# lh3/miniasm

Measured on NVIDIA H100. Metric: paf_overlaps_per_sec_ingest_to_gfa, higher is better.
Workload: dtype int64/uint32 (+3 float32 predicates)

## Files before the change

### miniasm_b200/csrc/capi_fused.cu

```cuda
#include "../../include/miniasm_b200.h"
#include "capi_util.cuh"
#include "hit_dev.cuh"
#include "clean_dev.cuh"
#include "gfa_dev.cuh"
#include "dump_dev.cuh"
#include "ugseq_dev.cuh"
#include <pthread.h>
#include "ingest_dev.cuh"
#include "shard_comm.cuh"
#include <cub/cub.cuh>
#include <map>
#include <string>
#include <zlib.h>
#include <fcntl.h>
#include <unistd.h>
#include <sys/stat.h>

ma_ug_t *mab_ug_download(MabDev &d, DUnitigs &du);
extern "C" sdict_t *sd_from_packed(char *block, size_t block_size, uint32_t n, const uint32_t *len);

struct mab_ctx {
	MabDev dev;
	char *d_text = nullptr;
	size_t text_len = 0, text_cap = 0;
// ... 279 lines not shown
	uint32_t *nl = (uint32_t*)malloc((dict->n_seq ? dict->n_seq : 1) * 4), *sl = (uint32_t*)malloc((dict->n_seq ? dict->n_seq : 1) * 4);
	bytes = 0;
	for (uint32_t i = 0; i < dict->n_seq; ++i) {
		size_t l = strlen(dict->seq[i].name);
		memcpy(pack + bytes, dict->seq[i].name, l + 1);
		off[i] = bytes, nl[i] = (uint32_t)l, sl[i] = dict->seq[i].len;
		bytes += l + 1;
	}
	text_reserve(c, bytes);
	c->text_len = bytes;
	DNames &nm = c->names;
	nm.n_seq = dict->n_seq;
	nm.off = mab_alloc<uint64_t>(d, nm.n_seq); nm.nlen = mab_alloc<uint32_t>(d, nm.n_seq); nm.slen = mab_alloc<uint32_t>(d, nm.n_seq);
	if (bytes) MAB_CUDA(cudaMemcpyAsync(c->d_text, pack, bytes, cudaMemcpyHostToDevice, d.stream));
	if (nm.n_seq) {
		MAB_CUDA(cudaMemcpyAsync(nm.off, off, (size_t)nm.n_seq * 8, cudaMemcpyHostToDevice, d.stream));
		MAB_CUDA(cudaMemcpyAsync(nm.nlen, nl, (size_t)nm.n_seq * 4, cudaMemcpyHostToDevice, d.stream));
		MAB_CUDA(cudaMemcpyAsync(nm.slen, sl, (size_t)nm.n_seq * 4, cudaMemcpyHostToDevice, d.stream));
	}
	d.sync();
	free(pack); free(off); free(nl); free(sl);
	c->n_seq = dict->n_seq;
	c->stats.n_hits_stored = n, c->stats.n_seq_in = dict->n_seq;
	return 0;
}

int mab_select(mab_ctx_t *c, const ma_opt_t *opt, int no_first, int no_second, int stage)
{
	MAB_CUDA(cudaSetDevice(c->dev.device));
	MabDev &d = c->dev;
	DHits &h = c->hits;
	PhaseTimer pt(d, &c->stats.ms_select, "mab_select");
	ctx_drop_graphs(c);
	auto step3_banner = [] { if (!mab_mute && ma_verbose >= 1) fprintf(stderr, "[M::main] ===> Step 3: 2-pass (fine) read selection <===\n"); };
	if (!no_first && !no_second && stage >= 5) {
		if (!mab_mute && ma_verbose >= 1) fprintf(stderr, "[M::main] ===> Step 2: 1-pass (crude) read selection <===\n");
		select_default(c, opt, { step3_banner });
		c->stats.n_hits_final = h.n, c->stats.n_seq_final = c->n_seq;
		d.sync();
		return 0;
	}
	if (!no_first) {
		if (!mab_mute && ma_verbose >= 1) fprintf(stderr, "[M::main] ===> Step 2: 1-pass (crude) read selection <===\n");
		if (stage >= 2) {
			d.free(c->sub);
			c->sub = mab_alloc<DSub>(d, c->n_seq);
			d.trace("select:begin");
			dh_sub(d, h, opt->min_dp, opt->min_iden, 0, c->sub);
			d.trace("select:sub1");
			dh_cut(d, h, c->sub, opt->min_span);
			if (stage >= 3) dh_flt(d, h, c->sub, (int)(opt->max_hang * 1.5), (int)(opt->min_ovlp * .5), &c->cov);
			d.trace("select:cut1(+flt)");
		}
	}
	if (!no_second) {
		step3_banner();
		if (stage >= 4) {
			DSub *sub2 = mab_alloc<DSub>(d, c->n_seq);
			d.trace("select:flt");
			dh_sub(d, h, opt->min_dp, opt->min_iden, opt->min_span / 2, sub2);
			d.trace("select:sub2");
			dh_cut(d, h, sub2, opt->min_span);
			if (!no_first && c->sub) { dh_sub_merge(d, c->n_seq, c->sub, sub2); d.free(sub2); }
			else { d.free(c->sub); c->sub = sub2; }
		}
		if (stage >= 5 && c->sub) {
// ... 110 lines not shown
	++d.n_lib;
	uint64_t last_pos; uint32_t last_sz;
	MAB_CUDA(cudaMemcpyAsync(&last_pos, pos + n - 1, 8, cudaMemcpyDeviceToHost, d.stream));
	MAB_CUDA(cudaMemcpyAsync(&last_sz, sz + n - 1, 4, cudaMemcpyDeviceToHost, d.stream));
	d.sync();
	const size_t bytes = last_pos + last_sz;
	char *d_pack = (char*)d.alloc(bytes), *pack = (char*)malloc(bytes);
	uint32_t *slen = (uint32_t*)malloc((size_t)n * 4);
	MAB_LAUNCH(d, k_name_pack, mab_grid(n, 256), 256, 0, n, c->orig_id, c->names.off, c->names.nlen, c->names.slen, c->name_text ? c->name_text : c->d_text, pos, d_pack, d_slen);
	MAB_CUDA(cudaMemcpyAsync(pack, d_pack, bytes, cudaMemcpyDeviceToHost, d.stream));
	MAB_CUDA(cudaMemcpyAsync(slen, d_slen, (size_t)n * 4, cudaMemcpyDeviceToHost, d.stream));
	d.sync();
	sd_destroy(dict);
	dict = sd_from_packed(pack, bytes, n, slen);
	free(slen);
	d.free(sz); d.free(d_slen); d.free(pos); d.free(d_pack);
	d.sync();
	return dict;
}

ma_sub_t *mab_export_sub(mab_ctx_t *c)
{
	MAB_CUDA(cudaSetDevice(c->dev.device));
	if (!c->sub) return 0;
	ma_sub_t *s = (ma_sub_t*)calloc(c->n_seq ? c->n_seq : 1, sizeof(ma_sub_t));
	if (c->n_seq) MAB_CUDA(cudaMemcpyAsync(s, c->sub, (size_t)c->n_seq * sizeof(DSub), cudaMemcpyDeviceToHost, c->dev.stream));
	c->dev.sync();
	return s;
}

ma_hit_t *mab_export_hits(mab_ctx_t *c, size_t *n)
{
	MAB_CUDA(cudaSetDevice(c->dev.device));
	ma_hit_t *a = (ma_hit_t*)malloc((c->hits.n ? c->hits.n : 1) * sizeof(ma_hit_t));
	if (c->hits.n) MAB_CUDA(cudaMemcpyAsync(a, c->hits.a, c->hits.n * sizeof(DHit), cudaMemcpyDeviceToHost, c->dev.stream));
	c->dev.sync();
	*n = c->hits.n;
	return a;
}

asg_t *mab_export_sg(mab_ctx_t *c)
{
	MAB_CUDA(cudaSetDevice(c->dev.device));
	if (!c->have_sg) return 0;
	asg_t *g = asg_init();
	g->n_seq = c->sg.n_seq, g->m_seq = c->sg.n_seq ? c->sg.n_seq : 1;
	g->seq = (asg_seq_t*)malloc((size_t)g->m_seq * sizeof(asg_seq_t));
	g->m_arc = c->sg.n_arc ? c->sg.n_arc : 1;
	g->arc = (asg_arc_t*)malloc((size_t)g->m_arc * sizeof(asg_arc_t));
	mab_graph_download(c->dev, c->sg, g);
	return g;
}

ma_ug_t *mab_export_ug(mab_ctx_t *c)
{
	MAB_CUDA(cudaSetDevice(c->dev.device));
	if (!c->have_ug) return 0;
	return mab_ug_download(c->dev, c->ug);
}

float mab_coverage(const mab_ctx_t *c) { return c->cov; }

long mab_write_gfa(mab_ctx_t *c, FILE *fp)
{
	MAB_CUDA(cudaSetDevice(c->dev.device));
	if (!c->have_ug) return -1;
	MabDev &d = c->dev;
	if (!c->ug.g.has_idx) dg_arc_index(d, c->ug.g);
	char *d_txt = nullptr;
	const size_t n = dg_gfa_text(d, c->ug, c->orig_id, c->names.off, c->names.nlen, c->name_text ? c->name_text : c->d_text, c->sub, &d_txt);
	if (n) {
		if (n > c->h_gfa_cap) {
			if (c->h_gfa) MAB_CUDA(cudaFreeHost(c->h_gfa));
			c->h_gfa_cap = n + (n >> 2) + (1 << 20);
			MAB_CUDA(cudaHostAlloc((void**)&c->h_gfa, c->h_gfa_cap, cudaHostAllocDefault));
		}
		MAB_CUDA(cudaMemcpyAsync(c->h_gfa, d_txt, n, cudaMemcpyDeviceToHost, d.stream));
		d.sync();
		if (fwrite(c->h_gfa, 1, n, fp) != n) { fprintf(stderr, "[E::miniasm_b200] short write of the GFA text\n"); exit(74); }
	}
	d.free(d_txt);
	d.sync();
	return (long)n;
}

static long write_dump(mab_ctx *c, DumpKind kind, uint64_t n_rec, FILE *fp)
{
	const DumpView v{{c->orig_id, c->names.off, c->names.nlen, c->name_text ? c->name_text : c->d_text, c->sub}, c->hits.a, c->sg.arc};
	return (long)dg_dump_write(c->dev, kind, v, n_rec, fp, c->pin, c->pin_bytes);
}

long mab_write_paf(mab_ctx_t *c, FILE *fp)
{
	MAB_CUDA(cudaSetDevice(c->dev.device));
	if (!c->sub) return -1;
	return write_dump(c, DUMP_PAF, c->hits.n, fp);
}

long mab_write_bed(mab_ctx_t *c, FILE *fp)
{
	MAB_CUDA(cudaSetDevice(c->dev.device));
	if (!c->sub) return -1;
	return write_dump(c, DUMP_BED, c->n_seq, fp);
}

long mab_write_sg(mab_ctx_t *c, FILE *fp)
{
	MAB_CUDA(cudaSetDevice(c->dev.device));
	if (!c->have_sg) return -1;
	return write_dump(c, DUMP_SG, c->sg.n_arc, fp);
}

static void *reads_loader(void *p)
{
	mab_ctx::ReadsLoad *rl = (mab_ctx::ReadsLoad*)p;
	const size_t CH = 32u << 20;
	cudaStream_t st;
	char *pin[2];
	cudaEvent_t ev[2];
	MAB_CUDA(cudaSetDevice(rl->device));
	gzFile fp = rl->fn != "-" ? gzopen(rl->fn.c_str(), "r") : gzdopen(fileno(stdin), "r");
	if (fp == 0) { rl->rc = -1; return 0; }
	gzbuffer(fp, 1 << 20);
	MAB_CUDA(cudaStreamCreateWithFlags(&st, cudaStreamNonBlocking));
	for (int i = 0; i < 2; ++i) { MAB_CUDA(cudaMallocHost(&pin[i], CH)); MAB_CUDA(cudaEventCreateWithFlags(&ev[i], cudaEventDisableTiming)); }
	struct stat sb;
	size_t guess = 0;
	if (rl->fn != "-" && stat(rl->fn.c_str(), &sb) == 0) guess = (size_t)sb.st_size;
// ... 134 lines not shown
	ctx_reset_reads(c);
	text_reserve(c, len);
	c->text_len = len;
	PhaseTimer pt(d, &c->stats.ms_ingest, "mab_load_ingest_text_sharded");
	ingest_paf_sharded(d, c->sc, c->d_text, c->text_len, min_span, min_match, bi_dir, c->hits, c->names, &c->name_text, c->ist, text);
	c->n_seq = c->names.n_seq;
	c->stats.n_lines = c->ist.n_parsed, c->stats.n_hits_stored = c->ist.n_hits, c->stats.n_seq_in = c->ist.n_seq;
	if (!mab_mute && ma_verbose >= 3 && c->sc.rank == 0)
		fprintf(stderr, "[M::%s::%s] read %ld hits; stored %ld hits and %d sequences (%ld bp)\n", "ma_hit_read", sys_timestamp(),
				(long)c->ist.n_parsed, (long)c->ist.n_hits, (int)c->ist.n_seq, (long)c->ist.tot_len);
	return 0;
}

static void sum_over_ranks(void *ctx, unsigned long long *v, int n)
{
	mab_ctx *c = (mab_ctx*)ctx;
	if (!c->sc.active() || n <= 0 || n > 8) return;
	MabDev &d = c->dev;
	unsigned long long *buf = (unsigned long long*)mab_alloc<uint64_t>(d, 8);
	MAB_CUDA(cudaMemcpyAsync(buf, v, 8 * (size_t)n, cudaMemcpyHostToDevice, d.stream));
	MAB_NCCL(ncclAllReduce(buf, buf, (size_t)n, ncclUint64, ncclSum, c->sc.comm, d.stream));
	MAB_CUDA(cudaMemcpyAsync(v, buf, 8 * (size_t)n, cudaMemcpyDeviceToHost, d.stream));
	d.sync();
	d.free(buf);
}

int mab_select_sharded(mab_ctx_t *c, const ma_opt_t *opt)
{
	MAB_CUDA(cudaSetDevice(c->dev.device));
	MabDev &d = c->dev;
	ShardComm &sc = c->sc;
	PhaseTimer pt(d, &c->stats.ms_select, "mab_select_sharded");
	ctx_drop_graphs(c);
	const int msave = mab_mute;
	if (sc.rank != 0) mab_mute = 1;
	mab_count_hook = sum_over_ranks, mab_count_hook_ctx = c;
	const uint32_t n = c->n_seq;
	SelectHooks hk;
	hk.sub_done = [&](DSub *s) { sc_allreduce(d, sc, s, n, ncclUint64, ncclSum); };
	hk.flags_done = [&](DSub *sub, uint8_t *used, uint32_t n_seq) {
		sc_allreduce(d, sc, sub, (size_t)n_seq * 2, ncclUint32, ncclMax);
		sc_allreduce(d, sc, used, n_seq, ncclUint8, ncclMax);
	};
	select_default(c, opt, hk);
	mab_mute = msave;
	mab_count_hook = nullptr, mab_count_hook_ctx = nullptr;
	c->stats.n_hits_final = c->hits.n, c->stats.n_seq_final = c->n_seq;
	d.sync();
	return 0;
}

__global__ void k_not_flag(const uint8_t *flag, uint32_t n, uint8_t *out)
{
	for (uint32_t i = blockIdx.x * blockDim.x + threadIdx.x; i < n; i += gridDim.x * blockDim.x) out[i] = !flag[i];
}

int mab_layout_sharded(mab_ctx_t *c, const ma_opt_t *opt)
{
	MAB_CUDA(cudaSetDevice(c->dev.device));
	MabDev &d = c->dev;
	ShardComm &sc = c->sc;
	const int G = sc.world;
	PhaseTimer pt(d, &c->stats.ms_layout, "mab_layout_sharded");
	ctx_drop_graphs(c);
	const int msave = mab_mute;
	if (sc.rank != 0) mab_mute = 1;
// ... 109 lines not shown
```

### miniasm_b200/csrc/hit_dev.cu

```cuda
#include "hit_dev.cuh"
#include "hit2arc.cuh"
#include <cub/cub.cuh>
#include <functional>

extern "C" int ma_verbose;
extern "C" const char *sys_timestamp(void);
#define ma_verbose_dev (mab_mute ? 0 : ma_verbose)

thread_local MabCountHook mab_count_hook = nullptr;
thread_local void *mab_count_hook_ctx = nullptr;
static inline void sum_ranks(unsigned long long *v, int n) { if (mab_count_hook) mab_count_hook(mab_count_hook_ctx, v, n); }

__device__ __forceinline__ DHit ld_hit(const DHit *p)
{
	const uint4 *q = reinterpret_cast<const uint4*>(p);
	uint4 a = __ldg(q), b = __ldg(q + 1);
	DHit h;
	h.qns = (uint64_t)a.y << 32 | a.x; h.qe = a.z; h.tn = a.w;
	h.ts = b.x; h.te = b.y; h.ml_rev = b.z; h.bl_del = b.w;
	return h;
}
__device__ __forceinline__ DHit ld_hit_rw(const DHit *p)
{
	const uint4 *q = reinterpret_cast<const uint4*>(p);
	uint4 a = q[0], b = q[1];
	DHit h;
	h.qns = (uint64_t)a.y << 32 | a.x; h.qe = a.z; h.tn = a.w;
	h.ts = b.x; h.te = b.y; h.ml_rev = b.z; h.bl_del = b.w;
	return h;
}
__device__ __forceinline__ void st_hit(DHit *p, const DHit &h)
{
	uint4 *q = reinterpret_cast<uint4*>(p);
	q[0] = make_uint4((uint32_t)h.qns, (uint32_t)(h.qns >> 32), h.qe, h.tn);
	q[1] = make_uint4(h.ts, h.te, h.ml_rev, h.bl_del);
}

static inline uint32_t bits_for(uint64_t x) { uint32_t b = 0; while (x) ++b, x >>= 1; return b ? b : 1; }

static void drop_bounds(MabDev &d, DHits &h) { d.free(h.grp); h.grp = nullptr; }

void dh_reserve(MabDev &d, DHits &h, size_t m)
{
	drop_bounds(d, h);
	if (m <= h.m) return;
	DHit *na = mab_alloc<DHit>(d, m), *nb = mab_alloc<DHit>(d, m);
	if (h.n) MAB_CUDA(cudaMemcpyAsync(na, h.a, h.n * sizeof(DHit), cudaMemcpyDeviceToDevice, d.stream));
	d.free(h.a); d.free(h.a2);
	h.a = na, h.a2 = nb, h.m = m;
}

void dh_free(MabDev &d, DHits &h)
{
	d.free(h.a); d.free(h.a2); d.free(h.grp);
	h = DHits();
}

constexpr int SEL_ROWS = 8, SEL_THREADS = 256, SEL_TILE = SEL_ROWS * SEL_THREADS;
static_assert(SEL_ROWS * (SEL_THREADS / 32) == 64, "k_sel_scatter scans exactly two counts per lane of one warp");

__global__ void __launch_bounds__(SEL_THREADS)
k_sel_count(const uint8_t *__restrict__ flag, size_t n, uint32_t *__restrict__ tile_cnt, unsigned long long *__restrict__ total)
{
	__shared__ unsigned s_w[SEL_THREADS / 32];
	const size_t base = (size_t)blockIdx.x * SEL_TILE;
	unsigned c = 0;
	#pragma unroll
	for (int k = 0; k < SEL_ROWS; ++k) {
		const size_t i = base + (size_t)k * SEL_THREADS + threadIdx.x;
		c += (i < n && flag[i] != 0) ? 1u : 0u;
	}
	c = __reduce_add_sync(0xffffffffu, c);
	if ((threadIdx.x & 31) == 0) s_w[threadIdx.x >> 5] = c;
	__syncthreads();
	if (threadIdx.x == 0) {
		unsigned t = 0;
		#pragma unroll
		for (int w = 0; w < SEL_THREADS / 32; ++w) t += s_w[w];
		tile_cnt[blockIdx.x] = t;
		if (t) atomicAdd(total, (unsigned long long)t);
	}
}

__global__ void __launch_bounds__(SEL_THREADS)
k_sel_scatter(const DHit *__restrict__ in, const uint8_t *__restrict__ flag, size_t n, const uint32_t *__restrict__ tile_off,
              DHit *__restrict__ out, unsigned long long *__restrict__ n_out)
{
// ... 1024 lines not shown
			DHit p;
			bool keep = false, dirty = false;
			if (i < end) {
				p = ld_hit_rw(a + i);
				const DHit o = p;
				const DSub rt = sub2[p.tn];
				keep = mab_cut_hit(p, rq, rt, min_span);
				if (keep) {
					dirty = hit_clipped(p, o);
					DArc tmp;
					const int rr = mab_hit2arc(p, (int)(rq.e - rq.s_del), (int)(rt.e - rt.s_del), hp.max_hang, hp.int_frac, hp.min_ovlp, &tmp);
					if (rr == MAB_HT_QCONT) atomicOr(&sub[r].s_del, MAB_DEL_BIT);
					else if (rr == MAB_HT_TCONT) atomicOr(&sub[p.tn].s_del, MAB_DEL_BIT);
					used[p.tn] = 1;
				}
			}
			const unsigned km = __ballot_sync(0xffffffffu, keep);
			const uint32_t dst = first + kept + __popc(km & lt);
			if (keep) {
				if (dst != i || dirty) st_hit(a + dst, p);
				tn_out[dst] = p.tn;
			}
			kept += __popc(km);
		}
		if (lane == 0) {
			grp[r] = kept ? (uint64_t)first << 32 | (first + kept) : 0;
			if (kept) used[r] = 1, cut += kept;
		}
	}
	if (lane == 0 && cut) atomicAdd(n_cut, (unsigned long long)cut);
}

__global__ void __launch_bounds__(256)
k_sel_final_count(const uint64_t *__restrict__ grp, const uint32_t *__restrict__ tn, const int32_t *__restrict__ map, uint32_t n_seq, uint32_t *cnt)
{
	const int lane = threadIdx.x & 31;
	for (uint32_t r = (blockIdx.x * blockDim.x + threadIdx.x) >> 5; r < n_seq; r += (gridDim.x * blockDim.x) >> 5) {
		const int32_t m = map[r];
		if (m < 0) continue;
		const uint64_t g = grp[r];
		const uint32_t end = (uint32_t)g, first = (uint32_t)(g >> 32);
		unsigned c = 0;
		if (end) for (uint32_t i = first + lane; i < end; i += 32) c += map[tn[i]] >= 0;
		c = __reduce_add_sync(0xffffffffu, c);
		if (lane == 0) cnt[m] = c;
	}
}

__global__ void __launch_bounds__(256)
k_sel_final_copy(const DHit *__restrict__ a, const uint64_t *__restrict__ grp, const int32_t *__restrict__ map, uint32_t n_seq,
                 const uint32_t *__restrict__ off, const uint32_t *__restrict__ n_new, DHit *__restrict__ out, uint64_t *__restrict__ grp_out,
                 unsigned long long *scal)
{
	const int lane = threadIdx.x & 31;
	const unsigned lt = (1u << lane) - 1u;
	if (blockIdx.x == 0 && threadIdx.x == 0) { const uint32_t nn = *n_new; scal[SCS_NSEQ] = nn, scal[SCS_NHITS] = off[nn]; }
	for (uint32_t r = (blockIdx.x * blockDim.x + threadIdx.x) >> 5; r < n_seq; r += (gridDim.x * blockDim.x) >> 5) {
		const int32_t m = map[r];
		if (m < 0) continue;
		if (lane == 0) { const uint32_t s = off[m], e = off[m + 1]; grp_out[m] = e > s ? (uint64_t)s << 32 | e : 0; }
		const uint64_t g = grp[r];
		const uint32_t end = (uint32_t)g, first = (uint32_t)(g >> 32);
		if (end == 0) continue;
		uint32_t o = off[m];
		for (uint32_t c = first; c < end; c += 32) {
			const uint32_t i = c + lane;
			DHit h;
			int32_t tn = -1;
			if (i < end) { h = ld_hit(a + i); tn = map[h.tn]; }
			const unsigned km = __ballot_sync(0xffffffffu, tn >= 0);
			if (tn >= 0) {
				h.qns = (uint64_t)(uint32_t)m << 32 | (uint32_t)h.qns, h.tn = (uint32_t)tn;
				st_hit(out + o + __popc(km & lt), h);
			}
			o += __popc(km);
		}
	}
}

static unsigned warp_grid(uint32_t n_seq, unsigned warps_per_block)
{
	const unsigned g = (n_seq + warps_per_block - 1) / warps_per_block;
	return g < 1 ? 1 : g < MAB_SMS * 32u ? g : MAB_SMS * 32u;
}

static void exclusive_sum(MabDev &d, const uint32_t *in, uint32_t *out, size_t n)
{
	size_t tb = 0;
	cub::DeviceScan::ExclusiveSum(nullptr, tb, in, out, (int64_t)n, d.stream);
	void *tmp = d.tmp(tb);
	cub::DeviceScan::ExclusiveSum(tmp, tb, in, out, (int64_t)n, d.stream);
	++d.n_lib;
}

size_t dh_select(MabDev &d, DHits &h, DSub *sub, const SelectParams &o, int32_t *map_out, float *cov, const SelectHooks &hk)
{
	const uint32_t n_seq = h.n_seq;
	if (h.n >= (1ull << 31)) { fprintf(stderr, "[E::miniasm_b200] more than 2^31 hits on one GPU\n"); exit(73); }
	if (!h.grp) {
		h.grp = mab_alloc<uint64_t>(d, n_seq);
		MAB_CUDA(cudaMemsetAsync(h.grp, 0, (size_t)n_seq * 8, d.stream));
		if (h.n) MAB_LAUNCH(d, k_group_bounds, mab_grid(h.n, 256), 256, 0, h.a, h.n, (uint32_t*)h.grp, nullptr);
	}
	dh_sub(d, h, o.min_dp, o.min_iden, 0, sub);
	if (hk.sub_done) hk.sub_done(sub);
	d.trace("select:sub1");

	const int clip = o.min_span / 2;
	DSub *sub2 = mab_alloc<DSub>(d, n_seq);
	uint32_t *big = mab_alloc<uint32_t>(d, n_seq);
	MAB_CUDA(cudaMemsetAsync(sub2, 0, (size_t)n_seq * sizeof(DSub), d.stream));
	d.zero_scal(0, SCS_NHITS + 1);
	MAB_LAUNCH(d, k_sel_cut_flt_sub, warp_grid(n_seq, SUBW_WARPS), SUBW_WARPS * 32, 0, h.a, h.grp, n_seq, sub, o.min_span, o.flt_max_hang, o.flt_min_ovlp,
	           o.min_dp, o.min_iden, (uint32_t)clip, sub2, big, d.d_scal);
	const uint32_t n_big = (uint32_t)d.get_scal(SC_BIG);
	{
		unsigned long long gv[4] = { d.h_scal[SCS_DP], d.h_scal[SCS_LEN], d.h_scal[SCS_CUT], d.h_scal[SCS_FLT] };
		sum_ranks(gv, 4);
		*cov = (float)((double)gv[0] / gv[1]);
		if (ma_verbose_dev >= 3) {
			fprintf(stderr, "[M::%s::%s] %ld hits remain after cut\n", "ma_hit_cut", sys_timestamp(), (long)gv[2]);
			fprintf(stderr, "[M::%s::%s] %ld hits remain after filtering; crude coverage after filtering: %.2f\n", "ma_hit_flt", sys_timestamp(), (long)gv[3], *cov);
		}
	}
	if (hk.step3) hk.step3();
	if (n_big) sub_big_reads(d, h, h.grp, big, n_big, o.min_dp, o.min_iden, clip, sub2);
	d.free(big);
	{
		unsigned long long v[1] = { d.get_scal(SC_COUNT) };
		sum_ranks(v, 1);
		if (ma_verbose_dev >= 3) fprintf(stderr, "[M::%s::%s] %ld query sequences remain after sub\n", "ma_hit_sub", sys_timestamp(), (long)v[0]);
	}
	if (hk.sub_done) hk.sub_done(sub2);
	dh_sub_merge(d, n_seq, sub, sub2);
	d.trace("select:cut1+flt+sub2");

	uint8_t *used = mab_alloc<uint8_t>(d, n_seq);
	uint32_t *tn = reinterpret_cast<uint32_t*>(h.a2);
	MAB_CUDA(cudaMemsetAsync(used, 0, n_seq, d.stream));
	MAB_LAUNCH(d, k_sel_cut_cont, warp_grid(n_seq, 8), 256, 0, h.a, h.grp, n_seq, sub2, sub, o.min_span, o.cont, used, tn, d.d_scal + SCS_CUT2);
	if (hk.flags_done) hk.flags_done(sub, used, n_seq);

	uint32_t *keep = mab_alloc<uint32_t>(d, (size_t)n_seq + 1), *excl = mab_alloc<uint32_t>(d, (size_t)n_seq + 1);
	uint32_t *cnt = mab_alloc<uint32_t>(d, (size_t)n_seq + 1), *off = mab_alloc<uint32_t>(d, (size_t)n_seq + 1);
	MAB_CUDA(cudaMemsetAsync(keep + n_seq, 0, 4, d.stream));
	MAB_LAUNCH(d, k_cont_keep, mab_grid(n_seq, 256), 256, 0, n_seq, sub, used, nullptr, keep);
	exclusive_sum(d, keep, excl, (size_t)n_seq + 1);
	MAB_LAUNCH(d, k_cont_map, mab_grid(n_seq, 256), 256, 0, n_seq, keep, excl, map_out, sub, sub2);
	MAB_LAUNCH(d, k_sel_final_count, warp_grid(n_seq, 8), 256, 0, h.grp, tn, map_out, n_seq, cnt);
	exclusive_sum(d, cnt, off, (size_t)n_seq + 1);
	uint64_t *grp_new = mab_alloc<uint64_t>(d, n_seq);
	MAB_LAUNCH(d, k_sel_final_copy, warp_grid(n_seq, 8), 256, 0, h.a, h.grp, map_out, n_seq, off, excl + n_seq, h.a2, grp_new, d.d_scal);
	const uint32_t n_new = (uint32_t)d.get_scal(SCS_NSEQ);
	const size_t n_hits = (size_t)d.h_scal[SCS_NHITS];
	const unsigned long long n_cut2 = d.h_scal[SCS_CUT2];
	if (n_new) MAB_CUDA(cudaMemcpyAsync(sub, sub2, (size_t)n_new * sizeof(DSub), cudaMemcpyDeviceToDevice, d.stream));
	d.free(sub2); d.free(used); d.free(keep); d.free(excl); d.free(cnt); d.free(off);
	DHit *t = h.a; h.a = h.a2; h.a2 = t;
	h.n = n_hits, h.n_seq = n_new;
	d.free(h.grp);
	h.grp = grp_new;
	d.trace("select:cut2+contained");

	unsigned long long gv[2] = { n_cut2, (unsigned long long)h.n };
	sum_ranks(gv, 2);
	if (ma_verbose_dev >= 3) {
		fprintf(stderr, "[M::%s::%s] %ld hits remain after cut\n", "ma_hit_cut", sys_timestamp(), (long)gv[0]);
		fprintf(stderr, "[M::%s::%s] %d sequences and %ld hits remain after containment removal\n", "ma_hit_contained", sys_timestamp(), n_new, (long)gv[1]);
	}
	return h.n;
}

__global__ void k_seq_set(uint32_t n_seq, const uint32_t *len, const uint8_t *del, uint32_t *seq, unsigned *max_len)
{
	unsigned mx = 0;
	for (uint32_t i = blockIdx.x * blockDim.x + threadIdx.x; i < n_seq; i += gridDim.x * blockDim.x) {
		uint32_t l = len[i] & 0x7fffffffu;
		seq[i] = l | (del && del[i] ? MAB_DEL_BIT : 0);
		mx = l > mx ? l : mx;
	}
	mx = __reduce_max_sync(0xffffffffu, mx);
	if ((threadIdx.x & 31) == 0 && mx) atomicMax(max_len, mx);
}

__global__ void k_sg_arcs(const DHit *a, size_t n, uint32_t *seq, HitArcParams p, uint32_t lb, uint64_t sentinel, uint64_t *key, uint64_t *val, unsigned long long *n_emit)
{
	unsigned cnt = 0;
	for (size_t i = blockIdx.x * (size_t)blockDim.x + threadIdx.x; i < n; i += (size_t)gridDim.x * blockDim.x) {
		DHit h = ld_hit(a + i);
		const uint32_t qn = (uint32_t)(h.qns >> 32);
		DArc t;
		t.ul = 0, t.v = 0, t.ol_del = 0;
		int r = mab_hit2arc(h, (int)(seq[qn] & 0x7fffffffu), (int)(seq[h.tn] & 0x7fffffffu), p.max_hang, p.int_frac, p.min_ovlp, &t);
		bool emit = false;
		if (r >= 0) {
			if (qn == h.tn) {
				if ((uint32_t)h.qns == h.ts && h.qe == h.te && (h.ml_rev >> 31)) atomicOr(&seq[qn], MAB_DEL_BIT);
			} else emit = true;
		} else if (r == MAB_HT_QCONT) atomicOr(&seq[qn], MAB_DEL_BIT);
		key[i] = emit ? ((t.ul >> 32) << lb | (uint32_t)t.ul) : sentinel;
		val[i] = (uint64_t)t.ol_del << 32 | t.v;
		cnt += emit;
	}
	cnt = __reduce_add_sync(0xffffffffu, cnt);
	if ((threadIdx.x & 31) == 0 && cnt) atomicAdd(n_emit, (unsigned long long)cnt);
}

constexpr int SGW_WARPS = 8, SGW_HITS = 256, SGW_IDX_BITS = 9;
constexpr int SGC_HITS = 8192, SGC_THREADS = 512;

typedef cub::ScanTileState<uint32_t> ArcTileState;
typedef cub::TilePrefixCallbackOp<uint32_t, ::cuda::std::plus<uint32_t>, ArcTileState> ArcPrefixOp;

__global__ void k_arc_tiles_init(ArcTileState ts, int n_tile) { ts.InitializeStatus(n_tile); }

__global__ void k_grp_max(const uint64_t *grp, uint32_t n, unsigned long long *mx)
{
	unsigned m = 0;
	for (uint32_t i = blockIdx.x * blockDim.x + threadIdx.x; i < n; i += gridDim.x * blockDim.x) {
		const uint64_t g = grp[i];
		const unsigned c = (uint32_t)g ? (uint32_t)g - (uint32_t)(g >> 32) : 0;
		m = c > m ? c : m;
	}
	m = __reduce_max_sync(0xffffffffu, m);
	if ((threadIdx.x & 31) == 0 && m) atomicMax(mx, (unsigned long long)m);
}

__global__ void __launch_bounds__(SGW_WARPS * 32)
k_sg_onepass(const DHit *__restrict__ a, const uint64_t *__restrict__ grp, uint32_t *seq, uint32_t n_seq, HitArcParams p, uint32_t lb,
             unsigned long long *tile_ctr, ArcTileState tstate, DArc *__restrict__ out, uint64_t *__restrict__ idx, uint2 *__restrict__ big_list,
             unsigned long long *scal)
{
	__shared__ uint32_t s_key[SGW_WARPS][SGW_HITS], s_v[SGW_WARPS][SGW_HITS], s_ol[SGW_WARPS][SGW_HITS];
	__shared__ typename ArcPrefixOp::TempStorage s_pref;
	__shared__ uint32_t s_n[SGW_WARPS], s_tile, s_base;
	const int warp = threadIdx.x >> 5, lane = threadIdx.x & 31;
	const unsigned lt = (1u << lane) - 1u;
	uint32_t *key = s_key[warp], *pv = s_v[warp], *pol = s_ol[warp];
	const uint32_t len_mask = (1u << lb) - 1u;
	if (threadIdx.x == 0) s_tile = (uint32_t)atomicAdd(tile_ctr, 1ull);
	__syncthreads();
	const uint32_t t = s_tile, r = t * SGW_WARPS + warp;
	uint32_t first = 0, cnt = 0, n = 0, n0 = 0;
	int ql = 0;
	if (r < n_seq) {
		const uint64_t g = grp[r];
		if ((uint32_t)g) first = (uint32_t)(g >> 32), cnt = (uint32_t)g - first;
		ql = (int)(seq[r] & 0x7fffffffu);
	}
	const bool big = cnt > SGW_HITS;
	for (uint32_t c = 0; c < cnt; c += 32) {
		bool ok = false;
		DArc e;
		e.ul = 0, e.v = 0, e.ol_del = 0;
		if (c + lane < cnt) {
			const DHit h = ld_hit(a + first + c + lane);
			const int rr = mab_hit2arc(h, ql, (int)(seq[h.tn] & 0x7fffffffu), p.max_hang, p.int_frac, p.min_ovlp, &e);
			if (rr >= 0) {
				if (h.tn == r) {
					if ((uint32_t)h.qns == h.ts && h.qe == h.te && (h.ml_rev >> 31)) atomicOr(&seq[r], MAB_DEL_BIT);
				} else ok = true;
			} else if (rr == MAB_HT_QCONT) atomicOr(&seq[r], MAB_DEL_BIT);
		}
		const uint32_t dir = (uint32_t)(e.ul >> 32) & 1u;
		const unsigned m = __ballot_sync(0xffffffffu, ok), m0 = __ballot_sync(0xffffffffu, ok && dir == 0);
		if (ok && !big) {
			const uint32_t k = n + __popc(m & lt);
			key[k] = ((dir << lb | (uint32_t)e.ul) << SGW_IDX_BITS) | k;
			pv[k] = e.v, pol[k] = e.ol_del;
		}
		n += __popc(m), n0 += __popc(m0);
	}
	if (n && !big) {
		uint32_t np = 32; while (np < n) np <<= 1;
		__syncwarp();
		switch (np) {
			case 32: sub_sort_regs<1>(key, n, lane); break;
			case 64: sub_sort_regs<2>(key, n, lane); break;
			case 128: sub_sort_regs<4>(key, n, lane); break;
			default: sub_sort_regs<8>(key, n, lane); break;
		}
		__syncwarp();
	}
	if (lane == 0) {
		s_n[warp] = n;
		if (r < n_seq && (atomicOr(&seq[r], 0u) & MAB_DEL_BIT)) atomicAdd(scal + SC_NSEL, 1ull);
	}
	__syncthreads();
	if (warp == 0) {
		const uint32_t agg = __reduce_add_sync(0xffffffffu, lane < SGW_WARPS ? s_n[lane] : 0u);
		if (t == 0) {
			if (lane == 0) tstate.SetInclusive(0, agg), s_base = 0;
		} else {
			ArcPrefixOp op(tstate, s_pref, ::cuda::std::plus<uint32_t>(), (int)t);
			const uint32_t ex = op(agg);
			if (lane == 0) s_base = ex;
		}
		if (lane == 0 && agg) atomicAdd(scal + SC_COUNT, (unsigned long long)agg);
	}
	__syncthreads();
	if (r >= n_seq) return;
	uint32_t base = s_base;
	for (int w = 0; w < warp; ++w) base += s_n[w];
	if (lane == 0) {
		idx[2 * (size_t)r] = n0 ? (uint64_t)base << 32 | n0 : 0;
		idx[2 * (size_t)r + 1] = n > n0 ? (uint64_t)(base + n0) << 32 | (n - n0) : 0;
		if (big && n) big_list[atomicAdd(scal + SC_BIG, 1ull)] = make_uint2(r, base);
	}
	if (big) return;
	for (uint32_t j = lane; j < n; j += 32) {
		const uint32_t k = key[j], src = k & ((1u << SGW_IDX_BITS) - 1u), kl = k >> SGW_IDX_BITS;
		*reinterpret_cast<uint4*>(out + base + j) = make_uint4(kl & len_mask, r << 1 | kl >> lb, pv[src], pol[src]);
	}
}

__global__ void __launch_bounds__(SGC_THREADS)
k_sg_sort_cta(const DHit *__restrict__ a, const uint64_t *__restrict__ grp, const uint32_t *__restrict__ seq,
              const uint2 *__restrict__ big_list, uint32_t n_big, HitArcParams p, DArc *__restrict__ out)
{
	typedef cub::BlockScan<uint32_t, SGC_THREADS> BS;
	extern __shared__ __align__(16) unsigned char sg_smem[];
	uint64_t *key = reinterpret_cast<uint64_t*>(sg_smem);
	uint32_t *pv = reinterpret_cast<uint32_t*>(key + SGC_HITS), *pol = pv + SGC_HITS;
	__shared__ typename BS::TempStorage s_scan;
	const uint32_t tid = threadIdx.x, nt = blockDim.x;
	for (uint32_t b = blockIdx.x; b < n_big; b += gridDim.x) {
		const uint2 rb = big_list[b];
		const uint32_t r = rb.x, base = rb.y;
		const uint64_t g = grp[r];
		const uint32_t first = (uint32_t)(g >> 32), cnt = (uint32_t)g - first;
		const int ql = (int)(seq[r] & 0x7fffffffu);
		uint32_t n = 0;
		for (uint32_t c0 = 0; c0 < cnt; c0 += nt) {
			const uint32_t c = c0 + tid;
			bool ok = false;
			DArc e;
			e.ul = 0, e.v = 0, e.ol_del = 0;
			if (c < cnt) {
				const DHit h = ld_hit(a + first + c);
				const int rr = mab_hit2arc(h, ql, (int)(seq[h.tn] & 0x7fffffffu), p.max_hang, p.int_frac, p.min_ovlp, &e);
				ok = rr >= 0 && h.tn != r;
			}
			uint32_t k, tot;
			BS(s_scan).ExclusiveSum((uint32_t)ok, k, tot);
			if (ok) {
				k += n;
				key[k] = (uint64_t)((((uint32_t)(e.ul >> 32) & 1u) << 31) | (uint32_t)e.ul) << 32 | k;
				pv[k] = e.v, pol[k] = e.ol_del;
			}
			n += tot;
			__syncthreads();
		}
		uint32_t np = 2; while (np < n) np <<= 1;
		for (uint32_t i = n + tid; i < np; i += nt) key[i] = ~0ull;
		__syncthreads();
		for (uint32_t k = 2, lk = 1; k <= np; k <<= 1, ++lk)
			for (uint32_t lj = lk; lj-- > 0;) {
				const uint32_t j = 1u << lj;
				for (uint32_t t = tid; t < np / 2; t += nt) {
					const uint32_t lo = ((t >> lj) << (lj + 1)) | (t & (j - 1)), hi = lo + j;
					const uint64_t x = key[lo], y = key[hi];
					const bool asc = (lo & k) == 0;
					if ((x > y) == asc) key[lo] = y, key[hi] = x;
				}
				__syncthreads();
			}
		for (uint32_t j = tid; j < n; j += nt) {
			const uint64_t k = key[j];
			const uint32_t src = (uint32_t)k, kl = (uint32_t)(k >> 32);
			*reinterpret_cast<uint4*>(out + base + j) = make_uint4(kl & 0x7fffffffu, r << 1 | kl >> 31, pv[src], pol[src]);
		}
		__syncthreads();
	}
}

static bool sg_emit_segmented(MabDev &d, const DHits &h, const HitArcParams &p, uint32_t lb, DGraph &g, uint32_t *n_del)
{
	const size_t n = h.n;
	const uint32_t n_seq = h.n_seq;
	if (lb + 1 + SGW_IDX_BITS > 32 || n >= (1ull << 31) || n_seq == 0) return false;
	d.zero_scal(SC_COUNT, 5);
	d.zero_scal(SC_NSEL);
	d.zero_scal(SC_TMP0);
	const uint64_t *grp = h.grp;
	uint64_t *own = nullptr;
	if (!grp) {
		own = mab_alloc<uint64_t>(d, n_seq);
		MAB_CUDA(cudaMemsetAsync(own, 0, (size_t)n_seq * 8, d.stream));
		MAB_LAUNCH(d, k_group_bounds, mab_grid(n, 256), 256, 0, h.a, n, (uint32_t*)own, d.d_scal + SC_AUX2);
		grp = own;
	}
	MAB_LAUNCH(d, k_grp_max, mab_grid(n_seq, 256), 256, 0, grp, n_seq, d.d_scal + SC_AUX);
	const bool ok = d.get_scal(SC_AUX) <= (unsigned long long)SGC_HITS && d.h_scal[SC_AUX2] == 0;
	if (ok) {
		dg_reserve(d, g, n);
		const int n_tile = (int)((n_seq + SGW_WARPS - 1) / SGW_WARPS);
		size_t ts_bytes = 0;
		MAB_CUDA(ArcTileState::AllocationSize(n_tile, ts_bytes));
		void *ts_mem = d.alloc(ts_bytes);
		ArcTileState ts;
		MAB_CUDA(ts.Init(n_tile, ts_mem, ts_bytes));
		MAB_LAUNCH(d, k_arc_tiles_init, mab_grid((size_t)n_tile, 256, 1u << 30), 256, 0, ts, n_tile);
		uint2 *big = mab_alloc<uint2>(d, n_seq);
		MAB_LAUNCH(d, k_sg_onepass, n_tile, SGW_WARPS * 32, 0, h.a, grp, g.seq, n_seq, p, lb, d.d_scal + SC_TMP0, ts, g.arc, g.idx, big, d.d_scal);
		g.n_arc = (uint32_t)d.get_scal(SC_COUNT);
		*n_del = (uint32_t)d.h_scal[SC_NSEL];
		const uint32_t n_big = (uint32_t)d.h_scal[SC_BIG];
		if (n_big) {
			const size_t smem = (size_t)SGC_HITS * 16;
			MAB_CUDA(cudaFuncSetAttribute(k_sg_sort_cta, cudaFuncAttributeMaxDynamicSharedMemorySize, (int)smem));
			MAB_LAUNCH(d, k_sg_sort_cta, n_big < MAB_SMS ? n_big : MAB_SMS, SGC_THREADS, smem, h.a, grp, g.seq, big, n_big, p, g.arc);
		}
		d.free(ts_mem); d.free(big);
		g.len_bits = lb, g.is_srt = true, g.has_idx = true;
	}
	d.free(own);
	return ok;
}

void dh_sg_gen(MabDev &d, const DHits &h, const uint32_t *len, const uint8_t *del, const HitArcParams &p, DGraph &g)
{
	const int64_t n_del = dh_sg_emit(d, h, len, del, p, g);
	if ((n_del < 0 ? dg_n_del_seq(d, g) : (uint32_t)n_del) != 0) dg_cleanup(d, g);
	else if (!g.has_idx) dg_arc_index(d, g);
	if (MAB_V(1)) fprintf(stderr, "[M::%s] read %d arcs\n", "ma_sg_gen", g.n_arc);
}

int64_t dh_sg_emit(MabDev &d, const DHits &h, const uint32_t *len, const uint8_t *del, const HitArcParams &p, DGraph &g)
{
	const uint32_t n_seq = h.n_seq;
	dg_set_nseq(d, g, n_seq);
	g.n_arc = 0, g.is_srt = false, g.is_symm = false, g.has_idx = false;
	d.zero_scal(SC_AUX);
	d.zero_scal(SC_COUNT);
	unsigned *d_max = (unsigned*)(d.d_scal + SC_AUX);
	if (n_seq) MAB_LAUNCH(d, k_seq_set, mab_grid(n_seq, 256), 256, 0, n_seq, len, del, g.seq, d_max);
	const unsigned mx = (unsigned)(d.get_scal(SC_AUX) & 0xffffffffu);
	const uint32_t lb = bits_for(mx);
	if (h.n) {
		if (h.n >= (1ull << 31)) { fprintf(stderr, "[E::miniasm_b200] more than 2^31 arcs on one GPU\n"); exit(73); }
		static const bool seg_sort = !(getenv("MAB_SG_SEGSORT") && atoi(getenv("MAB_SG_SEGSORT")) == 0);
		uint32_t n_del = 0;
		if (seg_sort && sg_emit_segmented(d, h, p, lb, g, &n_del)) return n_del;
		d.zero_scal(SC_COUNT);
		const uint64_t sentinel = 1ull << (lb + bits_for((uint64_t)n_seq * 2 - 1));
		uint64_t *ka = mab_alloc<uint64_t>(d, h.n), *kb = mab_alloc<uint64_t>(d, h.n), *va = mab_alloc<uint64_t>(d, h.n), *vb = mab_alloc<uint64_t>(d, h.n);
		MAB_LAUNCH(d, k_sg_arcs, mab_grid(h.n, 256), 256, 0, h.a, h.n, g.seq, p, lb, sentinel, ka, va, d.d_scal + SC_COUNT);
		const uint32_t n_arc = (uint32_t)d.get_scal(SC_COUNT);
		dg_build_sorted(d, g, ka, va, kb, vb, (uint32_t)h.n, n_arc, lb, true);
		d.free(ka); d.free(kb); d.free(va); d.free(vb);
	} else { dg_reserve(d, g, 1); g.is_srt = true; }
	return -1;
}
```

### miniasm_b200/csrc/hit_dev.cuh

```cuda
#pragma once
#include "mab_common.cuh"
#include "asg_dev.cuh"
#include <functional>

typedef void (*MabCountHook)(void *ctx, unsigned long long *v, int n);
extern thread_local MabCountHook mab_count_hook;
extern thread_local void *mab_count_hook_ctx;

struct DHits {
	DHit *a = nullptr, *a2 = nullptr;
	size_t n = 0, m = 0;
	uint32_t n_seq = 0;
	uint64_t *grp = nullptr;
};

struct HitArcParams { int max_hang; float int_frac; int min_ovlp; };

void dh_reserve(MabDev &d, DHits &h, size_t m);
void dh_free(MabDev &d, DHits &h);

void dh_sort(MabDev &d, DHits &h);
void dh_bucket_first(MabDev &d, const uint32_t *cnt, uint32_t n_seq, uint32_t *first);
void dh_sort_buckets(MabDev &d, DHits &h, const uint32_t *first);

uint64_t dh_sub(MabDev &d, const DHits &h, int min_dp, float min_iden, int end_clip, DSub *sub_out);

size_t dh_cut(MabDev &d, DHits &h, const DSub *reg, int min_span);

size_t dh_flt(MabDev &d, DHits &h, const DSub *sub, int max_hang, int min_ovlp, float *cov);

void dh_sub_merge(MabDev &d, uint32_t n_sub, DSub *a, const DSub *b);

size_t dh_contained(MabDev &d, DHits &h, DSub *sub, const uint8_t *seq_del, const HitArcParams &p, int32_t *map_out);
struct SelectParams { int min_dp; float min_iden; int min_span; int flt_max_hang, flt_min_ovlp; HitArcParams cont; };
struct SelectHooks {
	std::function<void()> step3;
	std::function<void(DSub*)> sub_done;
	std::function<void(DSub*, uint8_t*, uint32_t)> flags_done;
};
size_t dh_select(MabDev &d, DHits &h, DSub *sub, const SelectParams &o, int32_t *map_out, float *cov, const SelectHooks &hk);
int64_t dh_sg_emit(MabDev &d, const DHits &h, const uint32_t *len, const uint8_t *del, const HitArcParams &p, DGraph &g);

void dh_sg_gen(MabDev &d, const DHits &h, const uint32_t *len, const uint8_t *del, const HitArcParams &p, DGraph &g);
```

Before: 1.507 billion.

## Defer selected-hit compaction and fuse renumbering into string-graph emission

The final select step no longer copies surviving hits into a compacted array. It records the sequence map, offsets and new group bounds, and the onepass and sort-CTA string-graph kernels filter and renumber hits on the fly through a templated SEL path. The goal is to drop one full read and write pass over the hit array. The compaction still runs lazily through dh_hits_dense on export, PAF dump, reselection and the fallback emit path. In exchange, the graph kernels read from the uncompacted array, which adds a map lookup per hit and some wasted loads on dropped hits.

```diff
diff --git a/miniasm_b200/csrc/capi_fused.cu b/miniasm_b200/csrc/capi_fused.cu
--- a/miniasm_b200/csrc/capi_fused.cu
+++ b/miniasm_b200/csrc/capi_fused.cu
@@ -335,6 +335,7 @@
 	DHits &h = c->hits;
 	PhaseTimer pt(d, &c->stats.ms_select, "mab_select");
 	ctx_drop_graphs(c);
+	dh_hits_dense(d, h);
 	auto step3_banner = [] { if (!mab_mute && ma_verbose >= 1) fprintf(stderr, "[M::main] ===> Step 3: 2-pass (fine) read selection <===\n"); };
 	if (!no_first && !no_second && stage >= 5) {
 		if (!mab_mute && ma_verbose >= 1) fprintf(stderr, "[M::main] ===> Step 2: 1-pass (crude) read selection <===\n");
@@ -511,6 +512,7 @@
 ma_hit_t *mab_export_hits(mab_ctx_t *c, size_t *n)
 {
 	MAB_CUDA(cudaSetDevice(c->dev.device));
+	dh_hits_dense(c->dev, c->hits);
 	ma_hit_t *a = (ma_hit_t*)malloc((c->hits.n ? c->hits.n : 1) * sizeof(ma_hit_t));
 	if (c->hits.n) MAB_CUDA(cudaMemcpyAsync(a, c->hits.a, c->hits.n * sizeof(DHit), cudaMemcpyDeviceToHost, c->dev.stream));
 	c->dev.sync();
@@ -573,6 +575,7 @@
 {
 	MAB_CUDA(cudaSetDevice(c->dev.device));
 	if (!c->sub) return -1;
+	dh_hits_dense(c->dev, c->hits);
 	return write_dump(c, DUMP_PAF, c->hits.n, fp);
 }
 
@@ -773,6 +776,7 @@
 	ShardComm &sc = c->sc;
 	PhaseTimer pt(d, &c->stats.ms_select, "mab_select_sharded");
 	ctx_drop_graphs(c);
+	dh_hits_dense(d, c->hits);
 	const int msave = mab_mute;
 	if (sc.rank != 0) mab_mute = 1;
 	mab_count_hook = sum_over_ranks, mab_count_hook_ctx = c;
diff --git a/miniasm_b200/csrc/hit_dev.cu b/miniasm_b200/csrc/hit_dev.cu
--- a/miniasm_b200/csrc/hit_dev.cu
+++ b/miniasm_b200/csrc/hit_dev.cu
@@ -39,10 +39,12 @@
 static inline uint32_t bits_for(uint64_t x) { uint32_t b = 0; while (x) ++b, x >>= 1; return b ? b : 1; }
 
 static void drop_bounds(MabDev &d, DHits &h) { d.free(h.grp); h.grp = nullptr; }
+static void drop_selected(MabDev &d, DHits &h) { d.free(h.map); d.free(h.off); h.map = nullptr, h.off = nullptr; }
 
 void dh_reserve(MabDev &d, DHits &h, size_t m)
 {
 	drop_bounds(d, h);
+	drop_selected(d, h);
 	if (m <= h.m) return;
 	DHit *na = mab_alloc<DHit>(d, m), *nb = mab_alloc<DHit>(d, m);
 	if (h.n) MAB_CUDA(cudaMemcpyAsync(na, h.a, h.n * sizeof(DHit), cudaMemcpyDeviceToDevice, d.stream));
@@ -53,6 +55,7 @@
 void dh_free(MabDev &d, DHits &h)
 {
 	d.free(h.a); d.free(h.a2); d.free(h.grp);
+	drop_selected(d, h);
 	h = DHits();
 }
 
@@ -1143,7 +1146,8 @@
 }
 
 __global__ void __launch_bounds__(256)
-k_sel_final_count(const uint64_t *__restrict__ grp, const uint32_t *__restrict__ tn, const int32_t *__restrict__ map, uint32_t n_seq, uint32_t *cnt)
+k_sel_final_count(const uint64_t *__restrict__ grp, const uint32_t *__restrict__ tn, const int32_t *__restrict__ map, uint32_t n_seq, uint32_t *cnt,
+                  uint64_t *__restrict__ grp_out)
 {
 	const int lane = threadIdx.x & 31;
 	for (uint32_t r = (blockIdx.x * blockDim.x + threadIdx.x) >> 5; r < n_seq; r += (gridDim.x * blockDim.x) >> 5) {
@@ -1154,38 +1158,38 @@
 		unsigned c = 0;
 		if (end) for (uint32_t i = first + lane; i < end; i += 32) c += map[tn[i]] >= 0;
 		c = __reduce_add_sync(0xffffffffu, c);
-		if (lane == 0) cnt[m] = c;
-	}
+		if (lane == 0) cnt[m] = c, grp_out[m] = g;
+	}
+}
+
+__device__ __forceinline__ bool sel_renumber(DHit &h, uint32_t m, const int32_t *__restrict__ map)
+{
+	const int32_t tn = map[h.tn];
+	h.qns = (uint64_t)m << 32 | (uint32_t)h.qns, h.tn = (uint32_t)tn;
+	return tn >= 0;
 }
 
 __global__ void __launch_bounds__(256)
-k_sel_final_copy(const DHit *__restrict__ a, const uint64_t *__restrict__ grp, const int32_t *__restrict__ map, uint32_t n_seq,
-                 const uint32_t *__restrict__ off, const uint32_t *__restrict__ n_new, DHit *__restrict__ out, uint64_t *__restrict__ grp_out,
-                 unsigned long long *scal)
+k_sel_final_copy(const DHit *__restrict__ a, uint64_t *__restrict__ grp, const int32_t *__restrict__ map, uint32_t n_seq,
+                 const uint32_t *__restrict__ off, DHit *__restrict__ out)
 {
 	const int lane = threadIdx.x & 31;
 	const unsigned lt = (1u << lane) - 1u;
-	if (blockIdx.x == 0 && threadIdx.x == 0) { const uint32_t nn = *n_new; scal[SCS_NSEQ] = nn, scal[SCS_NHITS] = off[nn]; }
-	for (uint32_t r = (blockIdx.x * blockDim.x + threadIdx.x) >> 5; r < n_seq; r += (gridDim.x * blockDim.x) >> 5) {
-		const int32_t m = map[r];
-		if (m < 0) continue;
-		if (lane == 0) { const uint32_t s = off[m], e = off[m + 1]; grp_out[m] = e > s ? (uint64_t)s << 32 | e : 0; }
-		const uint64_t g = grp[r];
+	for (uint32_t m = (blockIdx.x * blockDim.x + threadIdx.x) >> 5; m < n_seq; m += (gridDim.x * blockDim.x) >> 5) {
+		const uint64_t g = grp[m];
 		const uint32_t end = (uint32_t)g, first = (uint32_t)(g >> 32);
-		if (end == 0) continue;
 		uint32_t o = off[m];
-		for (uint32_t c = first; c < end; c += 32) {
+		if (end) for (uint32_t c = first; c < end; c += 32) {
 			const uint32_t i = c + lane;
 			DHit h;
-			int32_t tn = -1;
-			if (i < end) { h = ld_hit(a + i); tn = map[h.tn]; }
-			const unsigned km = __ballot_sync(0xffffffffu, tn >= 0);
-			if (tn >= 0) {
-				h.qns = (uint64_t)(uint32_t)m << 32 | (uint32_t)h.qns, h.tn = (uint32_t)tn;
-				st_hit(out + o + __popc(km & lt), h);
-			}
+			bool live = false;
+			if (i < end) { h = ld_hit(a + i); live = sel_renumber(h, m, map); }
+			const unsigned km = __ballot_sync(0xffffffffu, live);
+			if (live) st_hit(out + o + __popc(km & lt), h);
 			o += __popc(km);
 		}
+		__syncwarp();
+		if (lane == 0) { const uint32_t s = off[m]; grp[m] = o > s ? (uint64_t)s << 32 | o : 0; }
 	}
 }
 
@@ -1202,6 +1206,16 @@
 	void *tmp = d.tmp(tb);
 	cub::DeviceScan::ExclusiveSum(tmp, tb, in, out, (int64_t)n, d.stream);
 	++d.n_lib;
+}
+
+void dh_hits_dense(MabDev &d, DHits &h)
+{
+	if (!h.map) return;
+	if (h.n_seq) {
+		MAB_LAUNCH(d, k_sel_final_copy, warp_grid(h.n_seq, 8), 256, 0, h.a, h.grp, h.map, h.n_seq, h.off, h.a2);
+		DHit *t = h.a; h.a = h.a2; h.a2 = t;
+	}
+	drop_selected(d, h);
 }
 
 size_t dh_select(MabDev &d, DHits &h, DSub *sub, const SelectParams &o, int32_t *map_out, float *cov, const SelectHooks &hk)
@@ -1254,23 +1268,26 @@
 
 	uint32_t *keep = mab_alloc<uint32_t>(d, (size_t)n_seq + 1), *excl = mab_alloc<uint32_t>(d, (size_t)n_seq + 1);
 	uint32_t *cnt = mab_alloc<uint32_t>(d, (size_t)n_seq + 1), *off = mab_alloc<uint32_t>(d, (size_t)n_seq + 1);
+	int32_t *map = mab_alloc<int32_t>(d, n_seq);
+	uint64_t *grp_new = mab_alloc<uint64_t>(d, n_seq);
 	MAB_CUDA(cudaMemsetAsync(keep + n_seq, 0, 4, d.stream));
+	MAB_CUDA(cudaMemsetAsync(cnt, 0, ((size_t)n_seq + 1) * 4, d.stream));
 	MAB_LAUNCH(d, k_cont_keep, mab_grid(n_seq, 256), 256, 0, n_seq, sub, used, nullptr, keep);
 	exclusive_sum(d, keep, excl, (size_t)n_seq + 1);
-	MAB_LAUNCH(d, k_cont_map, mab_grid(n_seq, 256), 256, 0, n_seq, keep, excl, map_out, sub, sub2);
-	MAB_LAUNCH(d, k_sel_final_count, warp_grid(n_seq, 8), 256, 0, h.grp, tn, map_out, n_seq, cnt);
+	MAB_LAUNCH(d, k_cont_map, mab_grid(n_seq, 256), 256, 0, n_seq, keep, excl, map, sub, sub2);
+	MAB_LAUNCH(d, k_sel_final_count, warp_grid(n_seq, 8), 256, 0, h.grp, tn, map, n_seq, cnt, grp_new);
 	exclusive_sum(d, cnt, off, (size_t)n_seq + 1);
-	uint64_t *grp_new = mab_alloc<uint64_t>(d, n_seq);
-	MAB_LAUNCH(d, k_sel_final_copy, warp_grid(n_seq, 8), 256, 0, h.a, h.grp, map_out, n_seq, off, excl + n_seq, h.a2, grp_new, d.d_scal);
+	MAB_CUDA(cudaMemcpyAsync(d.d_scal + SCS_NSEQ, excl + n_seq, 4, cudaMemcpyDeviceToDevice, d.stream));
+	MAB_CUDA(cudaMemcpyAsync(d.d_scal + SCS_NHITS, off + n_seq, 4, cudaMemcpyDeviceToDevice, d.stream));
+	if (n_seq) MAB_CUDA(cudaMemcpyAsync(map_out, map, (size_t)n_seq * 4, cudaMemcpyDeviceToDevice, d.stream));
 	const uint32_t n_new = (uint32_t)d.get_scal(SCS_NSEQ);
 	const size_t n_hits = (size_t)d.h_scal[SCS_NHITS];
 	const unsigned long long n_cut2 = d.h_scal[SCS_CUT2];
 	if (n_new) MAB_CUDA(cudaMemcpyAsync(sub, sub2, (size_t)n_new * sizeof(DSub), cudaMemcpyDeviceToDevice, d.stream));
-	d.free(sub2); d.free(used); d.free(keep); d.free(excl); d.free(cnt); d.free(off);
-	DHit *t = h.a; h.a = h.a2; h.a2 = t;
+	d.free(sub2); d.free(used); d.free(keep); d.free(excl); d.free(cnt);
 	h.n = n_hits, h.n_seq = n_new;
 	d.free(h.grp);
-	h.grp = grp_new;
+	h.grp = grp_new, h.map = map, h.off = off;
 	d.trace("select:cut2+contained");
 
 	unsigned long long gv[2] = { n_cut2, (unsigned long long)h.n };
@@ -1325,22 +1342,23 @@
 
 __global__ void k_arc_tiles_init(ArcTileState ts, int n_tile) { ts.InitializeStatus(n_tile); }
 
-__global__ void k_grp_max(const uint64_t *grp, uint32_t n, unsigned long long *mx)
+__global__ void k_grp_max(const uint64_t *grp, const uint32_t *off, uint32_t n, unsigned long long *mx)
 {
 	unsigned m = 0;
 	for (uint32_t i = blockIdx.x * blockDim.x + threadIdx.x; i < n; i += gridDim.x * blockDim.x) {
 		const uint64_t g = grp[i];
-		const unsigned c = (uint32_t)g ? (uint32_t)g - (uint32_t)(g >> 32) : 0;
+		const unsigned c = off ? off[i + 1] - off[i] : (uint32_t)g ? (uint32_t)g - (uint32_t)(g >> 32) : 0;
 		m = c > m ? c : m;
 	}
 	m = __reduce_max_sync(0xffffffffu, m);
 	if ((threadIdx.x & 31) == 0 && m) atomicMax(mx, (unsigned long long)m);
 }
 
+template <bool SEL>
 __global__ void __launch_bounds__(SGW_WARPS * 32)
-k_sg_onepass(const DHit *__restrict__ a, const uint64_t *__restrict__ grp, uint32_t *seq, uint32_t n_seq, HitArcParams p, uint32_t lb,
-             unsigned long long *tile_ctr, ArcTileState tstate, DArc *__restrict__ out, uint64_t *__restrict__ idx, uint2 *__restrict__ big_list,
-             unsigned long long *scal)
+k_sg_onepass(const DHit *__restrict__ a, const uint64_t *__restrict__ grp, const int32_t *__restrict__ map, uint32_t *seq, uint32_t n_seq,
+             HitArcParams p, uint32_t lb, unsigned long long *tile_ctr, ArcTileState tstate, DArc *__restrict__ out, uint64_t *__restrict__ idx,
+             uint2 *__restrict__ big_list, unsigned long long *scal)
 {
 	__shared__ uint32_t s_key[SGW_WARPS][SGW_HITS], s_v[SGW_WARPS][SGW_HITS], s_ol[SGW_WARPS][SGW_HITS];
 	__shared__ typename ArcPrefixOp::TempStorage s_pref;
@@ -1365,13 +1383,15 @@
 		DArc e;
 		e.ul = 0, e.v = 0, e.ol_del = 0;
 		if (c + lane < cnt) {
-			const DHit h = ld_hit(a + first + c + lane);
-			const int rr = mab_hit2arc(h, ql, (int)(seq[h.tn] & 0x7fffffffu), p.max_hang, p.int_frac, p.min_ovlp, &e);
-			if (rr >= 0) {
-				if (h.tn == r) {
-					if ((uint32_t)h.qns == h.ts && h.qe == h.te && (h.ml_rev >> 31)) atomicOr(&seq[r], MAB_DEL_BIT);
-				} else ok = true;
-			} else if (rr == MAB_HT_QCONT) atomicOr(&seq[r], MAB_DEL_BIT);
+			DHit h = ld_hit(a + first + c + lane);
+			if (!SEL || sel_renumber(h, r, map)) {
+				const int rr = mab_hit2arc(h, ql, (int)(seq[h.tn] & 0x7fffffffu), p.max_hang, p.int_frac, p.min_ovlp, &e);
+				if (rr >= 0) {
+					if (h.tn == r) {
+						if ((uint32_t)h.qns == h.ts && h.qe == h.te && (h.ml_rev >> 31)) atomicOr(&seq[r], MAB_DEL_BIT);
+					} else ok = true;
+				} else if (rr == MAB_HT_QCONT) atomicOr(&seq[r], MAB_DEL_BIT);
+			}
 		}
 		const uint32_t dir = (uint32_t)(e.ul >> 32) & 1u;
 		const unsigned m = __ballot_sync(0xffffffffu, ok), m0 = __ballot_sync(0xffffffffu, ok && dir == 0);
@@ -1425,8 +1445,9 @@
 	}
 }
 
+template <bool SEL>
 __global__ void __launch_bounds__(SGC_THREADS)
-k_sg_sort_cta(const DHit *__restrict__ a, const uint64_t *__restrict__ grp, const uint32_t *__restrict__ seq,
+k_sg_sort_cta(const DHit *__restrict__ a, const uint64_t *__restrict__ grp, const int32_t *__restrict__ map, const uint32_t *__restrict__ seq,
               const uint2 *__restrict__ big_list, uint32_t n_big, HitArcParams p, DArc *__restrict__ out)
 {
 	typedef cub::BlockScan<uint32_t, SGC_THREADS> BS;
@@ -1448,9 +1469,11 @@
 			DArc e;
 			e.ul = 0, e.v = 0, e.ol_del = 0;
 			if (c < cnt) {
-				const DHit h = ld_hit(a + first + c);
-				const int rr = mab_hit2arc(h, ql, (int)(seq[h.tn] & 0x7fffffffu), p.max_hang, p.int_frac, p.min_ovlp, &e);
-				ok = rr >= 0 && h.tn != r;
+				DHit h = ld_hit(a + first + c);
+				if (!SEL || sel_renumber(h, r, map)) {
+					const int rr = mab_hit2arc(h, ql, (int)(seq[h.tn] & 0x7fffffffu), p.max_hang, p.int_frac, p.min_ovlp, &e);
+					ok = rr >= 0 && h.tn != r;
+				}
 			}
 			uint32_t k, tot;
 			BS(s_scan).ExclusiveSum((uint32_t)ok, k, tot);
@@ -1501,7 +1524,7 @@
 		MAB_LAUNCH(d, k_group_bounds, mab_grid(n, 256), 256, 0, h.a, n, (uint32_t*)own, d.d_scal + SC_AUX2);
 		grp = own;
 	}
-	MAB_LAUNCH(d, k_grp_max, mab_grid(n_seq, 256), 256, 0, grp, n_seq, d.d_scal + SC_AUX);
+	MAB_LAUNCH(d, k_grp_max, mab_grid(n_seq, 256), 256, 0, grp, h.off, n_seq, d.d_scal + SC_AUX);
 	const bool ok = d.get_scal(SC_AUX) <= (unsigned long long)SGC_HITS && d.h_scal[SC_AUX2] == 0;
 	if (ok) {
 		dg_reserve(d, g, n);
@@ -1513,14 +1536,17 @@
 		MAB_CUDA(ts.Init(n_tile, ts_mem, ts_bytes));
 		MAB_LAUNCH(d, k_arc_tiles_init, mab_grid((size_t)n_tile, 256, 1u << 30), 256, 0, ts, n_tile);
 		uint2 *big = mab_alloc<uint2>(d, n_seq);
-		MAB_LAUNCH(d, k_sg_onepass, n_tile, SGW_WARPS * 32, 0, h.a, grp, g.seq, n_seq, p, lb, d.d_scal + SC_TMP0, ts, g.arc, g.idx, big, d.d_scal);
+		auto onepass = h.map ? k_sg_onepass<true> : k_sg_onepass<false>;
+		MAB_LAUNCH(d, onepass, n_tile, SGW_WARPS * 32, 0, h.a, grp, h.map, g.seq, n_seq, p, lb, d.d_scal + SC_TMP0, ts, g.arc, g.idx, big, d.d_scal);
 		g.n_arc = (uint32_t)d.get_scal(SC_COUNT);
 		*n_del = (uint32_t)d.h_scal[SC_NSEL];
 		const uint32_t n_big = (uint32_t)d.h_scal[SC_BIG];
 		if (n_big) {
 			const size_t smem = (size_t)SGC_HITS * 16;
-			MAB_CUDA(cudaFuncSetAttribute(k_sg_sort_cta, cudaFuncAttributeMaxDynamicSharedMemorySize, (int)smem));
-			MAB_LAUNCH(d, k_sg_sort_cta, n_big < MAB_SMS ? n_big : MAB_SMS, SGC_THREADS, smem, h.a, grp, g.seq, big, n_big, p, g.arc);
+			const unsigned grid = n_big < MAB_SMS ? n_big : MAB_SMS;
+			auto kern = h.map ? k_sg_sort_cta<true> : k_sg_sort_cta<false>;
+			MAB_CUDA(cudaFuncSetAttribute(kern, cudaFuncAttributeMaxDynamicSharedMemorySize, (int)smem));
+			MAB_LAUNCH(d, kern, grid, SGC_THREADS, smem, h.a, grp, h.map, g.seq, big, n_big, p, g.arc);
 		}
 		d.free(ts_mem); d.free(big);
 		g.len_bits = lb, g.is_srt = true, g.has_idx = true;
@@ -1529,7 +1555,7 @@
 	return ok;
 }
 
-void dh_sg_gen(MabDev &d, const DHits &h, const uint32_t *len, const uint8_t *del, const HitArcParams &p, DGraph &g)
+void dh_sg_gen(MabDev &d, DHits &h, const uint32_t *len, const uint8_t *del, const HitArcParams &p, DGraph &g)
 {
 	const int64_t n_del = dh_sg_emit(d, h, len, del, p, g);
 	if ((n_del < 0 ? dg_n_del_seq(d, g) : (uint32_t)n_del) != 0) dg_cleanup(d, g);
@@ -1537,7 +1563,7 @@
 	if (MAB_V(1)) fprintf(stderr, "[M::%s] read %d arcs\n", "ma_sg_gen", g.n_arc);
 }
 
-int64_t dh_sg_emit(MabDev &d, const DHits &h, const uint32_t *len, const uint8_t *del, const HitArcParams &p, DGraph &g)
+int64_t dh_sg_emit(MabDev &d, DHits &h, const uint32_t *len, const uint8_t *del, const HitArcParams &p, DGraph &g)
 {
 	const uint32_t n_seq = h.n_seq;
 	dg_set_nseq(d, g, n_seq);
@@ -1553,6 +1579,7 @@
 		static const bool seg_sort = !(getenv("MAB_SG_SEGSORT") && atoi(getenv("MAB_SG_SEGSORT")) == 0);
 		uint32_t n_del = 0;
 		if (seg_sort && sg_emit_segmented(d, h, p, lb, g, &n_del)) return n_del;
+		dh_hits_dense(d, h);
 		d.zero_scal(SC_COUNT);
 		const uint64_t sentinel = 1ull << (lb + bits_for((uint64_t)n_seq * 2 - 1));
 		uint64_t *ka = mab_alloc<uint64_t>(d, h.n), *kb = mab_alloc<uint64_t>(d, h.n), *va = mab_alloc<uint64_t>(d, h.n), *vb = mab_alloc<uint64_t>(d, h.n);
diff --git a/miniasm_b200/csrc/hit_dev.cuh b/miniasm_b200/csrc/hit_dev.cuh
--- a/miniasm_b200/csrc/hit_dev.cuh
+++ b/miniasm_b200/csrc/hit_dev.cuh
@@ -12,6 +12,8 @@
 	size_t n = 0, m = 0;
 	uint32_t n_seq = 0;
 	uint64_t *grp = nullptr;
+	int32_t *map = nullptr;
+	uint32_t *off = nullptr;
 };
 
 struct HitArcParams { int max_hang; float int_frac; int min_ovlp; };
@@ -39,6 +41,7 @@
 	std::function<void(DSub*, uint8_t*, uint32_t)> flags_done;
 };
 size_t dh_select(MabDev &d, DHits &h, DSub *sub, const SelectParams &o, int32_t *map_out, float *cov, const SelectHooks &hk);
-int64_t dh_sg_emit(MabDev &d, const DHits &h, const uint32_t *len, const uint8_t *del, const HitArcParams &p, DGraph &g);
+void dh_hits_dense(MabDev &d, DHits &h);
+int64_t dh_sg_emit(MabDev &d, DHits &h, const uint32_t *len, const uint8_t *del, const HitArcParams &p, DGraph &g);
 
-void dh_sg_gen(MabDev &d, const DHits &h, const uint32_t *len, const uint8_t *del, const HitArcParams &p, DGraph &g);
+void dh_sg_gen(MabDev &d, DHits &h, const uint32_t *len, const uint8_t *del, const HitArcParams &p, DGraph &g);
```

Measured after the change: 1.633 billion (median of 6 runs). +8.4%, better.
